# grayhong/self-diagnosing-gan

Hardware: AMD Instinct MI355X
Metric: images/sec (G+D step) (higher is better)
Workload: dtype f32

## Files before the change

### self-diagnosing-gan_amd/csrc/conv_wgrad.hip

```cpp
#include "conv_common.h"
#include "switches.h"
#include <stdlib.h>
#include <type_traits>


namespace diagan {
bool wgrad_wino_supported(int Hi, int Wi, int Ci, int Ho, int Wo, int Co, int R, int S, int sy, int dr, int off, int up,
                          int Kp);
int wgrad_wino_splits(int B, int Ho, int Wo, int Ci, int Co);
int launch_wgrad_wino(WgradArgs a, int splits, int segments, hipStream_t st);
int launch_wgrad_wino_batched(const WgradArgs* jobs, const int* splits, const int* segments, int n, hipStream_t st);
int wgrad_wino_batch_max();
bool wgrad_x3_takes(const WgradArgs& a, bool x3_on);
int launch_wgrad_x3(const WgradArgs& a, int splits, hipStream_t st);
void wgrad_x3_set(int on);


template <int BNn, int BNk, int PRO, bool P2>
__device__ __forceinline__ void conv_wgrad_body(const WgradArgs& a, const int bid, const int nblk) {
  constexpr int BK = 32;
  constexpr int TM = BNn / 64, TN = BNk / 64;
  constexpr int AC = BNn / 4, BC = BNk / 4;
  constexpr int AJ = BK * AC / 256, BJ = BK * BC / 256;
  constexpr int APR = 256 / AC, BPR = 256 / BC;
// ... 356 lines not shown
        for (int u = 0; u < U; ++u)
          t[u][r] = __builtin_bit_cast(f32x4, __builtin_amdgcn_raw_buffer_load_b128(src, voff[u] + (unsigned)r * sbytes, 0, 0));
#pragma unroll
      for (int u = 0; u < U; ++u) {
#pragma unroll
        for (int w = 1; w < R; w <<= 1)
#pragma unroll
          for (int r = 0; r + w < R; r += 2 * w) t[u][r] += t[u][r + w];
        acc[u] += t[u][0];
      }
    }
    if (sn) {
      double dot = 0.0;
      const __amdgpu_buffer_rsrc_t wsrc = __builtin_amdgcn_make_buffer_rsrc(const_cast<float*>(L.W), 0, L.n_w * 4, 0x00020000);
      const __amdgpu_buffer_rsrc_t dst = __builtin_amdgcn_make_buffer_rsrc(sl, 0, L.n_elem * 4, 0x00020000);
      f32x4 wv[U];
#pragma unroll
      for (int u = 0; u < U; ++u) wv[u] = __builtin_bit_cast(f32x4, __builtin_amdgcn_raw_buffer_load_b128(wsrc, voff[u], 0, 0));
#pragma unroll
      for (int u = 0; u < U; ++u) {
        const f32x4 g = acc[u];
        if (L.splits > 1)
          __builtin_amdgcn_raw_buffer_store_b128(__builtin_bit_cast(u32x4_t, g), dst, voff[u], 0, 0);
        dot += (double)g[0] * wv[u][0] + (double)g[1] * wv[u][1] + (double)g[2] * wv[u][2] + (double)g[3] * wv[u][3];
        acc[u] = z4;
      }
      dot = wave_sum(dot);
      __syncthreads();
      if ((threadIdx.x & 63) == 0) red[threadIdx.x >> 6] = dot;
      __syncthreads();
      if (threadIdx.x == 0) L.partials[c][lb] = (red[0] + red[1]) + (red[2] + red[3]);
    }
  }
  if (!sn) {
    const __amdgpu_buffer_rsrc_t gsrc = __builtin_amdgcn_make_buffer_rsrc(L.grad, 0, L.n_elem * 4, 0x00020000);
    f32x4 og[U];
#pragma unroll
    for (int u = 0; u < U; ++u) og[u] = __builtin_bit_cast(f32x4, __builtin_amdgcn_raw_buffer_load_b128(gsrc, voff[u], 0, 0));
#pragma unroll
    for (int u = 0; u < U; ++u)
      __builtin_amdgcn_raw_buffer_store_b128(__builtin_bit_cast(u32x4_t, og[u] + acc[u]), gsrc, voff[u], 0, 0);
  }
}

template <typename F>
__device__ __forceinline__ void fin_dispatch(int U, F&& f) {
  switch (U) {
    case 8: f(std::integral_constant<int, 8>{}); break;
    case 4: f(std::integral_constant<int, 4>{}); break;
    case 2: f(std::integral_constant<int, 2>{}); break;
    default: f(std::integral_constant<int, 1>{}); break;
  }
}

__global__ __launch_bounds__(256) __attribute__((amdgpu_waves_per_eu(4, 4))) void wgrad_finish_a_kernel(const WgFinish* __restrict__ tab, int n_layers) {
  const WgFinish L = load_uniform(tab + find_layer(tab, n_layers, blockIdx.x));
  const int lb = blockIdx.x - L.first_block;
  const int U = fin_u(L.splits);
  if ((long)lb * 1024 * U >= L.n_elem) return;
  __shared__ double red[4];
  fin_dispatch(U, [&](auto u) { fin_a<decltype(u)::value>(L, lb, red); });
}

__global__ __launch_bounds__(256) void wgrad_finish_dot_kernel(const WgFinish* __restrict__ tab) {
  const WgFinish L = tab[blockIdx.x];
  if (L.W == nullptr) return;
  __shared__ double red[256];
  const int fe = 1024 * fin_u(L.splits), nparts = (L.n_elem + fe - 1) / fe;
  for (int c = 0; c < L.nctx; ++c) {
    double d = 0.0;
    for (int k = threadIdx.x; k < nparts; k += 256) d += L.partials[c][k];
    red[threadIdx.x] = d;
    __syncthreads();
    for (int w = 128; w > 0; w >>= 1) {
      if ((int)threadIdx.x < w) red[threadIdx.x] += red[threadIdx.x + w];
      __syncthreads();
    }
    if (threadIdx.x == 0) L.partials[c][nparts] = red[0];
    __syncthreads();
  }
}

template <int U>
__device__ __forceinline__ void fin_b(const WgFinish& L, int lb) {
  constexpr int ELEMS = 1024 * U;
  constexpr int UC = U > 1 ? 2 : 1;
  const int nparts = (L.n_elem + ELEMS - 1) / ELEMS;
  float inv[2] = {0.f, 0.f}, coef[2] = {0.f, 0.f};
#pragma unroll
  for (int c = 0; c < 2; ++c) {
    if (c >= L.nctx) break;
    inv[c] = L.state[c][1];
    coef[c] = (float)(L.partials[c][nparts] * (double)inv[c]);
  }
  const int Co = L.n_w / L.Kp;
  const __amdgpu_buffer_rsrc_t gsrc = __builtin_amdgcn_make_buffer_rsrc(L.grad, 0, L.n_elem * 4, 0x00020000);
  __amdgpu_buffer_rsrc_t qsrc[2], vsrc[2], usrc[2];
#pragma unroll
  for (int c = 0; c < 2; ++c) {
    const bool on = c < L.nctx;
    qsrc[c] = __builtin_amdgcn_make_buffer_rsrc(L.slab[c], 0, on ? L.n_elem * 4 : 0, 0x00020000);
    vsrc[c] = __builtin_amdgcn_make_buffer_rsrc(const_cast<float*>(L.v[c]), 0, on ? L.Kp * 4 : 0, 0x00020000);
    usrc[c] = __builtin_amdgcn_make_buffer_rsrc(const_cast<float*>(L.u[c]), 0, on ? Co * 4 : 0, 0x00020000);
  }
#pragma unroll
  for (int u0 = 0; u0 < U; u0 += UC) {
    unsigned po[UC];
    bool okw[UC];
    f32x4 og[UC], gq[UC][2], vv[UC][2];
    float uu[UC][2];
#pragma unroll
    for (int i = 0; i < UC; ++i) {
      const long pos = (long)lb * ELEMS + ((u0 + i) * 256 + threadIdx.x) * 4;
      po[i] = pos < L.n_elem ? (unsigned)pos * 4u : 0x80000000u;
      okw[i] = pos < L.n_w;
      const unsigned n = okw[i] ? (unsigned)pos / (unsigned)L.Kp : 0u;
      const unsigned ko = okw[i] ? ((unsigned)pos - n * (unsigned)L.Kp) * 4u : 0x80000000u;
      const unsigned no = okw[i] ? n * 4u : 0x80000000u;
      og[i] = __builtin_bit_cast(f32x4, __builtin_amdgcn_raw_buffer_load_b128(gsrc, po[i], 0, 0));
#pragma unroll
      for (int c = 0; c < 2; ++c) {
        gq[i][c] = __builtin_bit_cast(f32x4, __builtin_amdgcn_raw_buffer_load_b128(qsrc[c], po[i], 0, 0));
        vv[i][c] = __builtin_bit_cast(f32x4, __builtin_amdgcn_raw_buffer_load_b128(vsrc[c], ko, 0, 0));
        uu[i][c] = __builtin_bit_cast(float, __builtin_amdgcn_raw_buffer_load_b32(usrc[c], no, 0, 0));
      }
    }
#pragma unroll
    for (int i = 0; i < UC; ++i) {
      f32x4 o = og[i];
#pragma unroll
      for (int c = 0; c < 2; ++c) {
        const f32x4 w = (gq[i][c] - (uu[i][c] * coef[c]) * vv[i][c]) * inv[c];
        o += okw[i] ? w : gq[i][c];
      }
      __builtin_amdgcn_raw_buffer_store_b128(__builtin_bit_cast(u32x4_t, o),
                                             gsrc, po[i], 0, 0);
    }
    __builtin_amdgcn_sched_barrier(0);
  }
}

__global__ __launch_bounds__(256) void wgrad_finish_b_kernel(const WgFinish* __restrict__ tab, int n_layers) {
  const WgFinish L = load_uniform(tab + find_layer(tab, n_layers, blockIdx.x));
  const int lb = blockIdx.x - L.first_block;
  const int U = fin_u(L.splits);
  if (L.W == nullptr || (long)lb * 1024 * U >= L.n_elem) return;
  fin_dispatch(U, [&](auto u) { fin_b<decltype(u)::value>(L, lb); });
}

extern "C" __attribute__((visibility("default"))) int diagan_wgrad_finish_block_elems(int splits) { return 1024 * fin_u(splits); }

}

using namespace diagan;
extern "C" int diagan_conv_gemm_get_wino(void);
extern "C" int diagan_conv_gemm_get_x3b(void);
extern "C" int diagan_conv_wgrad_splits(int M, int Co, int Kp);
extern "C" int diagan_conv_wgrad_uses_wino(int Hi, int Wi, int Ci, int Ho, int Wo, int Co, int R, int S, int sy, int dr,
                                           int off, int up, int Kp);

DIAGAN_API int diagan_wgrad_finish_batched(const void* table_dev, int n_layers, int64_t total_blocks, int any_sn,
                                           void* stream) {
  DG_REQUIRE(table_dev && n_layers > 0 && total_blocks > 0 && total_blocks < (1L << 31), "wgrad_finish_batched: bad args");
  static_assert(sizeof(WgFinish) == 128, "descriptor layout");
  const WgFinish* tab = (const WgFinish*)table_dev;
  hipStream_t st = (hipStream_t)stream;
  hipLaunchKernelGGL(wgrad_finish_a_kernel, dim3((unsigned)total_blocks), dim3(256), 0, st, tab, n_layers);
  if (any_sn) {
    hipLaunchKernelGGL(wgrad_finish_dot_kernel, dim3(n_layers), dim3(256), 0, st, tab);
    hipLaunchKernelGGL(wgrad_finish_b_kernel, dim3((unsigned)total_blocks), dim3(256), 0, st, tab, n_layers);
  }
  return check_launch("wgrad_finish_batched");
}

static void wgrad_tile(int Co, int Kp, int* bn, int* bk) {
  *bn = Co <= 64 ? 64 : 128;
  *bk = Kp <= 64 ? 64 : 128;
  if (*bn == 128 && *bk == 64) *bn = 64;
}

static void wgrad_gemm_fields(WgradArgs& a, int* bn, int* bk, bool* p2) {
  const ConvGeom& g = a.g;
  wgrad_tile(g.Co, g.Kp, bn, bk);
  a.tiles = cdiv(g.Co, *bn) * cdiv(g.Kp, *bk);
  a.same = (g.Hi == g.Ho && g.Wi == g.Wo && g.sy == 1 && g.up == 1) ? 1 : 0;
  *p2 = (g.Ho & (g.Ho - 1)) == 0 && (g.Wo & (g.Wo - 1)) == 0;
  a.lgW = a.lgHW = 0;
  while ((1 << a.lgW) < g.Wo) ++a.lgW;
  while ((1 << a.lgHW) < g.Ho * g.Wo) ++a.lgHW;
}

static int wgrad_fill_args(WgradArgs& a, const float* dy, const float* x, float* slab, int splits, int segments,
                           int64_t slab_stride, int64_t bias_off, const float* pro_scale, const float* pro_shift, int pro_mode, int B,
                           int Hi, int Wi, int Ci, int Ho, int Wo, int Co, int R, int S, int sy, int dr, int off, int up, int Kp) {
  DG_REQUIRE(dy && x && slab, "conv_wgrad: null tensor");
  DG_REQUIRE(B > 0 && Hi > 0 && Wi > 0 && Ho > 0 && Wo > 0 && R > 0 && S > 0, "conv_wgrad: bad dims");
  DG_REQUIRE(Ci > 0 && (Ci & 3) == 0 && Co > 0 && (Co & 3) == 0, "conv_wgrad: Ci=%d, Co=%d must be multiples of 4", Ci, Co);
  DG_REQUIRE(up == 1 || up == 2, "conv_wgrad: up=%d unsupported", up);
  DG_REQUIRE(dr == 1 || dr == -1, "conv_wgrad: dr must be +-1");
  DG_REQUIRE(Kp % 32 == 0 && Kp >= R * S * Ci, "conv_wgrad: bad Kp=%d", Kp);
  DG_REQUIRE(splits >= 1, "conv_wgrad: splits=%d", splits);
  DG_REQUIRE(pro_mode >= 0 && pro_mode <= PRO_BOX_RELU, "conv_wgrad: bad pro_mode %d", pro_mode);
  DG_REQUIRE(!(pro_mode == PRO_BOX || pro_mode == PRO_BOX_RELU) || (up == 1 && dr == 1 && Hi >= 2 && Wi >= 2),
             "conv_wgrad: the box-sum loader (pro_mode 5 / 6) gathers forward geometries without up-sampling");
  DG_REQUIRE(!(pro_mode == PRO_AFFINE_RELU || pro_mode == PRO_AFFINE) || (pro_scale && pro_shift),
             "conv_wgrad: affine prologue needs scale/shift");
  DG_REQUIRE(slab_stride >= (int64_t)Co * Kp && (bias_off < 0 || bias_off + Co <= slab_stride),
             "conv_wgrad: slab_stride=%ld too small for Co*Kp=%ld (+bias)", (long)slab_stride, (long)Co * Kp);
  DG_REQUIRE((long)Co * Kp * 4 < (1L << 31), "conv_wgrad: weight tensor must be smaller than 2 GiB");
  DG_REQUIRE((long)B * Ho * Wo * Co * 4 < (1L << 31) && (long)B * Hi * Wi * Ci * 4 < (1L << 31),
             "conv_wgrad: tensors must be smaller than 2 GiB (32-bit buffer offsets)");
  a.dy = dy; a.x = x; a.slab = slab; a.pro_scale = pro_scale; a.pro_shift = pro_shift; a.pro_mode = pro_mode;
  a.M = B * Ho * Wo;
  a.g = ConvGeom{B, Hi, Wi, Ci, Ho, Wo, Co, R, S, sy, dr, off, up, R * S * Ci, Kp};
  a.dWo = make_fastdiv((unsigned)Wo);
  a.dHo = make_fastdiv((unsigned)Ho);
  a.adv_b = 32 / (Ho * Wo);
  a.adv_y = (32 % (Ho * Wo)) / Wo;
  a.adv_x = (32 % (Ho * Wo)) % Wo;
  const int total_steps = cdiv(a.M, 32);
  DG_REQUIRE(segments >= 1 && splits % segments == 0, "conv_wgrad: splits=%d not a multiple of segments=%d", splits, segments);
  DG_REQUIRE(segments == 1 || (a.M % (32 * segments)) == 0, "conv_wgrad: %d pixels do not split into %d segments of whole K-steps", a.M, segments);
  a.seg_steps = cdiv(total_steps, segments);
  a.splits_per_seg = splits / segments;
  a.steps_per_split = cdiv(a.seg_steps, a.splits_per_seg);
  a.slab_stride = slab_stride;
  a.bias_off = bias_off;
  return DIAGAN_OK;
}

DIAGAN_API int diagan_conv_wgrad(const float* dy, const float* x, float* slab, int splits, int segments,
                                 int64_t slab_stride, int64_t bias_off, const float* pro_scale, const float* pro_shift, int pro_mode, int B,
                                 int Hi, int Wi, int Ci, int Ho, int Wo, int Co, int R, int S, int sy,
                                 int dr, int off, int up, int Kp, void* stream) {
  WgradArgs a;
  const int rc = wgrad_fill_args(a, dy, x, slab, splits, segments, slab_stride, bias_off, pro_scale, pro_shift, pro_mode, B, Hi, Wi, Ci,
                                 Ho, Wo, Co, R, S, sy, dr, off, up, Kp);
  if (rc != DIAGAN_OK) return rc;
  hipStream_t st = (hipStream_t)stream;
  if (diagan_conv_wgrad_uses_wino(Hi, Wi, Ci, Ho, Wo, Co, R, S, sy, dr, off, up, Kp))
    return launch_wgrad_wino(a, splits, segments, st);
  int bn, bk;
  bool p2;
  wgrad_gemm_fields(a, &bn, &bk, &p2);
  if (bn == 128 && bk == 128 && wgrad_x3_takes(a, diagan_conv_gemm_get_x3b() != 0)) return launch_wgrad_x3(a, splits, st);
  const dim3 grid(a.tiles * splits);
#define DG_WG(BN_, PRO_) do { if (p2) hipLaunchKernelGGL((conv_wgrad_kernel<BN_, 128, PRO_, true>), grid, dim3(256), 0, st, a); \
                              else hipLaunchKernelGGL((conv_wgrad_kernel<BN_, 128, PRO_, false>), grid, dim3(256), 0, st, a); } while (0)
#define DG_WG_ALL(BN_) switch (pro_mode) { \
      case PRO_NONE: DG_WG(BN_, PRO_NONE); break; \
      case PRO_RELU: DG_WG(BN_, PRO_RELU); break; \
// ... 156 lines not shown
```

### self-diagnosing-gan_amd/diagan/models/base.py

```python
import os

import torch

from diagan.models.layers import FlatNet
from diagan.ops import eltwise as E


PREFETCH_FAKES = os.environ.get("DIAGAN_PREFETCH_FAKES", "1") != "0"
STACK_G_STEP = os.environ.get("DIAGAN_STACK_G_STEP", "1") != "0"


def _world_size():
    from diagan.trainer import distributed as dist
    return dist.get_world_size()


class BaseModel(FlatNet):

    def restore_checkpoint(self, ckpt_file, optimizer=None):
        if not ckpt_file:
            raise ValueError("No checkpoint file to be restored.")
        ckpt_dict = torch.load(ckpt_file, map_location='cpu', weights_only=False)
        self.load_state_dict(ckpt_dict['model_state_dict'])
        self.param_version += 1
# ... 73 lines not shown
            return
        noise = [torch.randn((batch_size, self.nz), device=device) for _ in range(count)]
        for lo in range(0, count, per_chunk):
            part = noise[lo: lo + per_chunk]
            imgs, _ = self.forward_nhwc(torch.cat(part), True, save=False, groups=len(part))
            self._fake_pool.extend(imgs.split(batch_size))
        self._fake_pool_version = self.param_version

    def _take_prefetched(self, num_images):
        pool = getattr(self, '_fake_pool', None)
        if not pool:
            return None
        if pool[0].shape[0] != num_images or self._fake_pool_version != self.param_version or not self.training:
            self._fake_pool = []
            return None
        return pool.pop(0)

    def compute_gan_loss(self, output):
        k = None
        if getattr(self, 'use_topk', False):
            k = int(self.topk_rate * output.shape[0])
        errG, _ = E.loss_gen(output.detach().contiguous(), self.loss_type, k=k, need_grad=False)
        return errG[0]

    def adversarial_grads(self, real_batch, netD, optG, device=None, noise=None):
        self.zero_grad()
        self.wgrad_batch.hold = _world_size() > 1
        batch_size = real_batch[0].shape[0]
        fake, gctx = self.generate_images_nhwc(batch_size, device=device, noise=noise, save=True)
        output, dctx = netD.forward_nhwc(fake, netD.training, save=True, need_dgrad=True, need_in_dgrad=True)
        k = None
        if getattr(self, 'use_topk', False):
            k = int(self.topk_rate * batch_size)
        errG, dlogit = E.loss_gen(output, self.loss_type, k=k)
        g_img = netD.backward_nhwc(dctx, dlogit, need_wgrad=False, need_gx=True)
        self.backward_nhwc(gctx, g_img)
        self.sync_grads(optG)
        return errG

    def train_step(self, real_batch, netD, optG, log_data, device=None, global_step=None, scaler=None, noise=None,
                   **kwargs):
        if scaler is not None:
            raise NotImplementedError("amp/GradScaler is not part of the fp32 MI355X path")
        errG = self.adversarial_grads(real_batch, netD, optG, device=device, noise=noise)
        optG.step()
        log_data.add_metric('errG', errG[0], group='loss')
        return log_data


class BaseDiscriminator(BaseModel):
    supports_defer_step = True

    def __init__(self, ndf, loss_type, **kwargs):
        super().__init__()
        self.ndf, self.loss_type = ndf, loss_type
        self.use_gold = False

    def to_nhwc(self, x):
        return E.nchw_to_nhwc(x.to(dtype=torch.float32), self.in_channels_padded)

    def forward(self, x):
        logit, _ = self.forward_nhwc(self.to_nhwc(x), self.training, save=False, need_dgrad=False)
        return logit

    def compute_gan_loss(self, output_real, output_fake):
        out3, _, _ = E.loss_dis(output_real.detach().contiguous(), output_fake.detach().contiguous(),
                                self.loss_type, gold=self.use_gold, need_grad=False)
        return out3[0]

    def compute_probs(self, output_real, output_fake):
        out3, _, _ = E.loss_dis(output_real.detach().contiguous(), output_fake.detach().contiguous(),
                                self.loss_type, gold=False, need_grad=False)
        return out3[1].item(), out3[2].item()

    def train_step(self, real_batch, netG, optD, log_data, device=None, global_step=None, scaler=None, noise=None,
                   **kwargs):
        if scaler is not None:
            raise NotImplementedError("amp/GradScaler is not part of the fp32 MI355X path")
        self.zero_grad()
        self.wgrad_batch.hold = _world_size() > 1
        real_images = real_batch[0]
        batch_size = real_images.shape[0]
        if getattr(self, 'pair_forward', False) and self.training:
            B, _, H, W = real_images.shape
            x_all = torch.empty((2 * B, H, W, self.in_channels_padded), dtype=torch.float32, device=real_images.device)
            E.nchw_to_nhwc(real_images.to(dtype=torch.float32), self.in_channels_padded, out=x_all[:B])
            netG.generate_images_nhwc(batch_size, device=device, noise=noise, save=False, out=x_all[B:])
            out_all, ctx = self.forward_nhwc(x_all, True, save=True, need_dgrad=True, need_in_dgrad=False, slot='pair')
            dl = torch.empty(2 * B, dtype=torch.float32, device=x_all.device)
            out3, _, _ = E.loss_dis(out_all[:B], out_all[B:], self.loss_type, gold=self.use_gold, d_real=dl[:B],
                                    d_fake=dl[B:])
            self.backward_nhwc(ctx, dl, need_wgrad=True, need_gx=False)
        else:
            out_real, ctx_r = self.forward_nhwc(self.to_nhwc(real_images), self.training, save=True, need_dgrad=True,
                                                need_in_dgrad=False)
            fake, _ = netG.generate_images_nhwc(batch_size, device=device, noise=noise, save=False)
            out_fake, ctx_f = self.forward_nhwc(fake, self.training, save=True, need_dgrad=True, need_in_dgrad=False,
                                                slot=1)
            out3, d_real, d_fake = E.loss_dis(out_real, out_fake, self.loss_type, gold=self.use_gold)
            self.backward_nhwc(ctx_r, d_real, need_wgrad=True, need_gx=False)
            self.backward_nhwc(ctx_f, d_fake, need_wgrad=True, need_gx=False)
        defer = bool(kwargs.get('defer_step', False))
        self.sync_grads(optD, async_op=defer)
        if not defer:
            optD.step()
        log_data.add_metric('errD', out3[0], group='loss')
        log_data.add_metric('D(x)', out3[1], group='prob')
        log_data.add_metric('D(G(z))', out3[2], group='prob')
        return log_data
```

### self-diagnosing-gan_amd/diagan/models/sngan.py

```python
import math

import torch.nn as nn

from diagan.models.base import BaseDiscriminator, BaseGenerator
from diagan.models.layers import BatchNorm, ConvLayer, HeadLinear, LatentLinear, SNBatch
from diagan.ops import conv as C
from diagan.ops import eltwise as E

RELU = (C.PRO_RELU, None, None)


def _bn_pro(bn):
    return (C.PRO_AFFINE_RELU, bn.scale, bn.shift, bn.group_imgs)


class GBlock(nn.Module):
    def __init__(self, in_channels, out_channels, hidden_channels=None, upsample=False):
        super().__init__()
        hidden_channels = hidden_channels if hidden_channels is not None else out_channels
        self.learnable_sc = in_channels != out_channels or upsample
        self.upsample = upsample
        self.c1 = ConvLayer('conv', in_channels, hidden_channels, 3, 1, 1)
        self.c2 = ConvLayer('conv', hidden_channels, out_channels, 3, 1, 1)
        self.b1 = BatchNorm(in_channels)
# ... 68 lines not shown
class DBlock(nn.Module):

    def __init__(self, in_channels, out_channels, hidden_channels=None, downsample=False):
        super().__init__()
        hidden_channels = hidden_channels if hidden_channels is not None else in_channels
        self.downsample = downsample
        self.learnable_sc = (in_channels != out_channels) or downsample
        self.c1 = ConvLayer('conv', in_channels, hidden_channels, 3, 1, 1, sn=True)
        self.c2 = ConvLayer('conv', hidden_channels, out_channels, 3, 1, 1, sn=True)
        self.c1.xavier_(math.sqrt(2.0))
        self.c2.xavier_(math.sqrt(2.0))
        if self.learnable_sc:
            self.c_sc = ConvLayer('conv', in_channels, out_channels, 1, 1, 0, sn=True)
            self.c_sc.xavier_(1.0)

    def forward(self, x, training, save=True, need_dgrad=True, slot=None):
        k1 = self.c1.prepare(training, need_dgrad, slot)
        k2 = self.c2.prepare(training, need_dgrad, slot)
        h1 = self.c1.fwd(k1, x, pro=RELU)
        xp = None
        lo_ok = (x.shape[0] * (x.shape[1] // 2) * (x.shape[2] // 2)) % 64 == 0
        if self.learnable_sc and self.downsample and lo_ok:
            ksc = self.c_sc.prepare(training, need_dgrad, slot)
            xp = E.avgpool2(x, relu_in=True)
            sc = self.c_sc.fwd(ksc, xp)
            out = self.c2.fwd_pool(k2, h1, pro=RELU, residual=sc)
        elif self.learnable_sc:
            ksc = self.c_sc.prepare(training, need_dgrad, slot)
            sc = self.c_sc.fwd(ksc, x, pro=RELU)
            h2 = self.c2.fwd(k2, h1, pro=RELU, residual=sc)
            out = E.avgpool2(h2) if self.downsample else h2
        else:
            ksc = None
            h2 = self.c2.fwd(k2, h1, pro=RELU, residual=x, res_relu=True)
            out = E.avgpool2(h2) if self.downsample else h2
        ctx = dict(x=x, xp=xp, h1=h1, k1=k1, k2=k2, ksc=ksc, slot=0 if slot is None else slot) if save else {}
        return out, ctx

    def backward(self, ctx, gout, need_wgrad=True, need_gx=True):
        x, xp, h1, slot = ctx['x'], ctx['xp'], ctx['h1'], ctx['slot']
        hw = x.shape[1:3]
        unpool = self.downsample and self.c2.dgrad_unpool_fused(gout.shape[0], hw)
        pooled_w = self.downsample and need_wgrad and self.c2.wgrad_pooled_ok(gout, h1)
        lo_path = xp is not None
        need_full = self.downsample and ((need_wgrad and not pooled_w) or not unpool or not lo_path)
        g_full = E.avgpool2_bwd(gout) if need_full else gout
        if pooled_w:
            self.c2.wgrad_pooled(ctx['k2'], gout, h1, relu_in=True, slot=slot)
        elif need_wgrad:
            self.c2.wgrad(ctx['k2'], g_full, h1, pro=RELU, slot=slot)
        if unpool:
            g_h1 = self.c2.dgrad_unpool(ctx['k2'], gout, hw, mask_src=h1)
        else:
            g_h1 = self.c2.dgrad(ctx['k2'], g_full, hw, mask_src=h1)
        if need_wgrad:
            self.c1.wgrad(ctx['k1'], g_h1, x, pro=RELU, slot=slot)
            if xp is not None:
                self.c_sc.wgrad(ctx['ksc'], gout, xp, slot=slot)
            elif self.learnable_sc:
                self.c_sc.wgrad(ctx['ksc'], g_full, x, pro=RELU, slot=slot)
        if not need_gx:
            return None
        if xp is not None:
            g_xp = self.c_sc.dgrad(ctx['ksc'], gout, xp.shape[1:3])
            if self.c1.dgrad_res_unpool_fused(x.shape[0], hw):
                return self.c1.dgrad(ctx['k1'], g_h1, hw, residual=g_xp, mask_src=x, res_unpool=True)
            return self.c1.dgrad(ctx['k1'], g_h1, hw, residual=E.avgpool2_bwd(g_xp), mask_src=x)
        if self.learnable_sc:
            tmp = self.c_sc.dgrad(ctx['ksc'], g_full, hw)
            return self.c1.dgrad(ctx['k1'], g_h1, hw, residual=tmp, mask_src=x)
        return self.c1.dgrad(ctx['k1'], g_h1, hw, residual=g_full, mask_src=x)


class DBlockOptimized(nn.Module):
    def __init__(self, in_channels, out_channels):
        super().__init__()
        self.c1 = ConvLayer('conv', in_channels, out_channels, 3, 1, 1, sn=True)
        self.c2 = ConvLayer('conv', out_channels, out_channels, 3, 1, 1, sn=True)
        self.c_sc = ConvLayer('conv', in_channels, out_channels, 1, 1, 0, sn=True)
        self.c1.xavier_(math.sqrt(2.0))
        self.c2.xavier_(math.sqrt(2.0))
        self.c_sc.xavier_(1.0)

    def forward(self, x, training, save=True, need_dgrad=True, need_in_dgrad=False, slot=None):
        k1 = self.c1.prepare(training, need_dgrad and need_in_dgrad, slot)
        k2 = self.c2.prepare(training, need_dgrad, slot)
        ksc = self.c_sc.prepare(training, need_dgrad and need_in_dgrad, slot)
        h1 = self.c1.fwd(k1, x)
        xp = E.avgpool2(x)
        sc = self.c_sc.fwd(ksc, xp)
        out = self.c2.fwd_pool(k2, h1, pro=RELU, residual=sc)
        ctx = dict(x=x, xp=xp, h1=h1, k1=k1, k2=k2, ksc=ksc, slot=0 if slot is None else slot) if save else {}
        return out, ctx

    def backward(self, ctx, gout, need_wgrad=True, need_gx=True):
        x, xp, h1, slot = ctx['x'], ctx['xp'], ctx['h1'], ctx['slot']
        hw = x.shape[1:3]
        unpool = self.c2.dgrad_unpool_fused(gout.shape[0], hw)
        pooled_w = need_wgrad and self.c2.wgrad_pooled_ok(gout, h1)
        g_full = E.avgpool2_bwd(gout) if ((need_wgrad and not pooled_w) or not unpool) else None
        if need_wgrad:
            self.c_sc.wgrad(ctx['ksc'], gout, xp, slot=slot)
            if pooled_w:
                self.c2.wgrad_pooled(ctx['k2'], gout, h1, relu_in=True, slot=slot)
            else:
                self.c2.wgrad(ctx['k2'], g_full, h1, pro=RELU, slot=slot)
        if unpool:
            g_h1 = self.c2.dgrad_unpool(ctx['k2'], gout, hw, mask_src=h1)
        else:
            g_h1 = self.c2.dgrad(ctx['k2'], g_full, hw, mask_src=h1)
        if need_wgrad:
            self.c1.wgrad(ctx['k1'], g_h1, x, slot=slot)
        if not need_gx:
            return None
        g_xp = self.c_sc.dgrad(ctx['ksc'], gout, xp.shape[1:3])
        g_sc_full = E.avgpool2_bwd(g_xp)
        return self.c1.dgrad(ctx['k1'], g_h1, hw, residual=g_sc_full)


class SNGANBaseGenerator(BaseGenerator):
    out_channels = 3
    supports_stacked_forward = True

    def _blocks(self):
        raise NotImplementedError

    def forward_nhwc(self, z, training, save=True, out=None, groups=1, save_group=None):
        z = z.to(dtype=self.l1.weight.dtype)
        self.wino_batch(('f', None)).prepare(self.param_version)
        x0, h = self.l1.fwd(z)
        bctx = []
        blocks = self._blocks()
        bn = None
        for i, blk in enumerate(blocks):
            nxt = blocks[i + 1].b1 if i + 1 < len(blocks) else self._last_bn
            h, c, bn = blk.forward(h, training, save=save, need_dgrad=save, bn1=bn, next_bn=nxt, groups=groups,
                                   save_group=save_group)
            bctx.append(c)
        k = self._last_conv.prepare(training, need_dgrad=save)
        y_pre = self._last_conv.fwd(k, h, pro=_bn_pro(bn))
        y = E.tanh_fwd(y_pre, out=out)
        if save and groups > 1:
            b = z.shape[0] // groups
            sl = slice(save_group * b, (save_group + 1) * b)
            ctx = dict(x0=x0[sl], bctx=bctx, h=h[sl], bn=E.bn_ctx_group(bn, save_group), k=k, y=y[sl])
        else:
            ctx = dict(x0=x0, bctx=bctx, h=h, bn=bn, k=k, y=y) if save else None
        return y, ctx

    def backward_nhwc(self, ctx, g_img):
        g_pre = E.tanh_bwd(ctx['y'], g_img)
        self.wino_batch(('d', None)).prepare(self.param_version)
        h = ctx['h']
        self._last_conv.wgrad(ctx['k'], g_pre, h, pro=_bn_pro(ctx['bn']))
        g_a = self._last_conv.dgrad(ctx['k'], g_pre, h.shape[1:3])
        g = self._last_bn.bwd(g_a, h, ctx['bn'], relu=True)
        for blk, c in zip(reversed(self._blocks()), reversed(ctx['bctx'])):
            g = blk.backward(c, g)
        self.l1.wgrad(ctx['x0'], g)
        self.wgrad_batch.finish(0)


class SNGANGenerator32(SNGANBaseGenerator):
    max_stacked_images = 1536

    def __init__(self, nz=128, ngf=256, bottom_width=4, loss_type='hinge', **kwargs):
        super().__init__(nz=nz, ngf=ngf, bottom_width=bottom_width, loss_type=loss_type, **kwargs)
        self.l1 = LatentLinear(nz, ngf, bottom_width)
        self.block2 = GBlock(ngf, ngf, upsample=True)
        self.block3 = GBlock(ngf, ngf, upsample=True)
        self.block4 = GBlock(ngf, ngf, upsample=True)
        self.b5 = BatchNorm(ngf)
        self.c5 = ConvLayer('conv', ngf, 3, 3, 1, 1)
        self.l1.xavier_(1.0)
        self.c5.xavier_(1.0)
        self._link_layers()

    def _blocks(self):
        return [self.block2, self.block3, self.block4]

    @property
    def _last_bn(self):
        return self.b5

    @property
    def _last_conv(self):
        return self.c5


class SNGANGenerator64(SNGANBaseGenerator):
    max_stacked_images = 768

    def __init__(self, nz=128, ngf=1024, bottom_width=4, loss_type='hinge', **kwargs):
        super().__init__(nz=nz, ngf=ngf, bottom_width=bottom_width, loss_type=loss_type, **kwargs)
        self.l1 = LatentLinear(nz, ngf, bottom_width)
        self.block2 = GBlock(ngf, ngf >> 1, upsample=True)
        self.block3 = GBlock(ngf >> 1, ngf >> 2, upsample=True)
        self.block4 = GBlock(ngf >> 2, ngf >> 3, upsample=True)
        self.block5 = GBlock(ngf >> 3, ngf >> 4, upsample=True)
        self.b6 = BatchNorm(ngf >> 4)
        self.c6 = ConvLayer('conv', ngf >> 4, 3, 3, 1, 1)
        self.l1.xavier_(1.0)
        self.c6.xavier_(1.0)
        self._link_layers()

    def _blocks(self):
        return [self.block2, self.block3, self.block4, self.block5]

    @property
    def _last_bn(self):
        return self.b6

    @property
    def _last_conv(self):
        return self.c6


class SNGANBaseDiscriminator(BaseDiscriminator):
    in_channels_padded = 4
    pair_forward = True

    def _blocks(self):
        raise NotImplementedError

    def _sn_prepare(self, slot, training, need_dgrad):
        sb = getattr(self, '_sn_batch', None)
        if sb is None or sb.stale():
            layers = [m for m in self.modules() if isinstance(m, ConvLayer) and m.sn] + [self._head]
            sb = SNBatch(self, layers)
            object.__setattr__(self, '_sn_batch', sb)
        if slot == 'pair':
            sb.run_pair(training, need_dgrad)
        else:
            sb.run(slot, training, 1 if need_dgrad else 0)

    def forward_nhwc(self, x, training, save=True, need_dgrad=True, need_in_dgrad=True, slot=0):
        self._sn_prepare(slot, training, need_dgrad)
        self.wino_batch(('f', slot)).prepare(self._wino_version(slot))
        blocks = self._blocks()
        h, c0 = blocks[0].forward(x, training, save=save, need_dgrad=need_dgrad, need_in_dgrad=need_in_dgrad,
                                  slot=slot)
        bctx = [c0]
        for blk in blocks[1:]:
            h, c = blk.forward(h, training, save=save, need_dgrad=need_dgrad, slot=slot)
            bctx.append(c)
        hctx, logit = self._head.fwd(h, training, slot=slot)
        return logit, (dict(bctx=bctx, hctx=hctx, slot=slot) if save else None)

    def _wino_version(self, slot):
        sb = self._sn_batch
        return ('p', self.param_version) if slot == 'pair' else sb.slot_ver.get(slot)

    def backward_nhwc(self, ctx, dlogit, need_wgrad=True, need_gx=False):
        self.wino_batch(('d', ctx['slot'])).prepare(self._wino_version(ctx['slot']))
        g = self._head.bwd(ctx['hctx'], dlogit, need_wgrad=need_wgrad)
        blocks = self._blocks()
        for i in range(len(blocks) - 1, -1, -1):
            g = blocks[i].backward(ctx['bctx'][i], g, need_wgrad=need_wgrad, need_gx=(need_gx or i > 0))
        if need_wgrad:
            self.wgrad_batch.finish(ctx['slot'])
        return g


class SNGANDiscriminator32(SNGANBaseDiscriminator):
    def __init__(self, ndf=128, loss_type='hinge', **kwargs):
        super().__init__(ndf=ndf, loss_type=loss_type, **kwargs)
        self.block1 = DBlockOptimized(3, ndf)
        self.block2 = DBlock(ndf, ndf, downsample=True)
        self.block3 = DBlock(ndf, ndf, downsample=False)
        self.block4 = DBlock(ndf, ndf, downsample=False)
        self.l5 = HeadLinear(ndf, sn=True)
        self.l5.xavier_(1.0)
        self._link_layers()

    def _blocks(self):
        return [self.block1, self.block2, self.block3, self.block4]

    @property
    def _head(self):
        return self.l5


class SNGANDiscriminator64(SNGANBaseDiscriminator):
    def __init__(self, ndf=1024, loss_type='hinge', **kwargs):
        super().__init__(ndf=ndf, loss_type=loss_type, **kwargs)
        self.block1 = DBlockOptimized(3, ndf >> 4)
        self.block2 = DBlock(ndf >> 4, ndf >> 3, downsample=True)
        self.block3 = DBlock(ndf >> 3, ndf >> 2, downsample=True)
        self.block4 = DBlock(ndf >> 2, ndf >> 1, downsample=True)
        self.block5 = DBlock(ndf >> 1, ndf, downsample=True)
        self.l6 = HeadLinear(ndf, sn=True)
        self.l6.xavier_(1.0)
        self._link_layers()

    def _blocks(self):
        return [self.block1, self.block2, self.block3, self.block4, self.block5]

    @property
    def _head(self):
        return self.l6
```

### self-diagnosing-gan_amd/diagan/ops/eltwise.py

```python
import torch

from diagan import _native as nat

LOSS_TYPES = {'gan': 0, 'ns': 1, 'hinge': 2, 'wasserstein': 3}
ptr, st = nat.ptr, nat.current_stream


def _f32(shape, dev):
    return torch.empty(shape, dtype=torch.float32, device=dev)


_ws = {}
_ws_retired = []


def _workspace(dev, nbytes):
    w = _ws.get(dev.index)
    if w is None or w.numel() < nbytes:
        if w is not None:
            _ws_retired.append(w)
        w = torch.empty(max(int(nbytes), 1 << 20), dtype=torch.uint8, device=dev)
        _ws[dev.index] = w
    return w

# ... 60 lines not shown
    ws = _colred_ws(x.device, Mg, C, groups) if training else None
    if training and groups > 1:
        nat.call("diagan_bn_stats_grouped", ptr(x), Mg, C, groups, ptr(gamma), ptr(beta), eps, momentum, ptr(running_mean),
                 ptr(running_var), ptr(ctx.mean), ptr(ctx.invstd), ptr(ctx.scale), ptr(ctx.shift), ptr(ws), st())
        return ctx
    for g in range(groups):
        o = g * C * 4
        nat.call("diagan_bn_stats", ptr(x) + g * Mg * C * 4, Mg, C, ptr(gamma), ptr(beta), eps, momentum,
                 ptr(running_mean), ptr(running_var), 1 if training else 0, ptr(ctx.mean) + o, ptr(ctx.invstd) + o,
                 ptr(ctx.scale) + o, ptr(ctx.shift) + o, ptr(ws), st())
    return ctx


def bn_stats_fused(partials, tiles, M, gamma, beta, running_mean, running_var, eps=1e-5, momentum=0.1, groups=1,
                   group_imgs=0):
    C = gamma.numel()
    if tiles % groups or M % groups:
        raise RuntimeError(f"bn_stats_fused: {tiles} tiles / {M} rows do not split into {groups} groups")
    tg, Mg = tiles // groups, M // groups
    ctx = _bn_ctx(C, Mg, True, groups, group_imgs, gamma.device)
    splits = nat.fn("diagan_bn_stats_fused_splits")(tg, C, groups)
    ws = torch.empty(groups * splits * 2 * C, dtype=torch.float64, device=gamma.device) if splits > 1 else None
    nat.call("diagan_bn_stats_fused", ptr(partials), tg, Mg, C, ptr(gamma), ptr(beta), eps, momentum,
             ptr(running_mean), ptr(running_var), ptr(ctx.mean), ptr(ctx.invstd), ptr(ctx.scale), ptr(ctx.shift), groups,
             ptr(ws), 0 if ws is None else ws.numel(), st())
    return ctx


def bn_bwd(g, x, ctx, relu, dgamma, dbeta, accumulate, residual=None, slope=0.0, drop=None, drop_scale=1.0):
    dx = torch.empty_like(x)
    coef = _f32((2 * ctx.C,), x.device)
    ws = _colred_ws(x.device, ctx.M, ctx.C)
    nat.call("diagan_bn_bwd", ptr(g), ptr(x), ctx.M, ctx.C, ptr(ctx.scale), ptr(ctx.shift), ptr(ctx.mean),
             ptr(ctx.invstd), 1 if ctx.training else 0, 1 if relu else 0, slope, ptr(drop), drop_scale, ptr(dgamma), ptr(dbeta), 1 if accumulate else 0,
             ptr(residual),
             ptr(dx), ptr(coef), ptr(ws), st())
    return dx


def colsum(x, out, accumulate):
    C = x.shape[-1]
    M = x.numel() // C
    ws = _colred_ws(x.device, M, C)
    nat.call("diagan_colsum", ptr(x), M, C, ptr(out), 1 if accumulate else 0, ptr(ws), st())
    return out


def upsample2x(x, pro=None):
    B, H, W, C = x.shape
    mode, scale, shift, group_imgs = (tuple(pro) + (0,))[:4] if pro is not None else (0, None, None, 0)
    out = _f32((B, 2 * H, 2 * W, C), x.device)
    nat.call("diagan_upsample2x", ptr(x), ptr(out), B, H, W, C, mode, ptr(scale), ptr(shift), group_imgs, st())
    return out


def upsample2x_bwd(g, residual=None):
    B, H2, W2, C = g.shape
    out = _f32((B, H2 // 2, W2 // 2, C), g.device)
    nat.call("diagan_upsample2x_bwd", ptr(g), ptr(out), B, H2 // 2, W2 // 2, C, ptr(residual), st())
    return out


def boxsum2(x, relu_in=False):
    B, H, W, C = x.shape
    out = _f32((B, H + 1, W + 1, C), x.device)
    nat.call("diagan_boxsum2", ptr(x), ptr(out), B, H, W, C, 1 if relu_in else 0, st())
    return out


def avgpool2(x, residual=None, relu_in=False):
    B, H, W, C = x.shape
    out = _f32((B, H // 2, W // 2, C), x.device)
    nat.call("diagan_avgpool2", ptr(x), ptr(out), B, H, W, C, ptr(residual), 1 if relu_in else 0, st())
    return out


def avgpool2_bwd(g, residual=None):
    B, Ho, Wo, C = g.shape
    out = _f32((B, 2 * Ho, 2 * Wo, C), g.device)
    nat.call("diagan_avgpool2_bwd", ptr(g), ptr(out), B, 2 * Ho, 2 * Wo, C, ptr(residual), st())
    return out


def head_fwd(x, w, inv_sigma, bias, inv_sigma1=None):
    B, H, W, C = x.shape
    pooled = _f32((B, C), x.device)
    logit = _f32((B, 1), x.device)
    nat.call("diagan_head_fwd", ptr(x), ptr(w), ptr(inv_sigma), ptr(inv_sigma1), B // 2, ptr(bias), ptr(pooled),
             ptr(logit), B, H * W, C, st())
    return pooled, logit


def head_bwd(dlogit, w, inv_sigma, x, pooled, need_gx=True, need_wgrad=True, dbias=None, accumulate_bias=True,
             inv_sigma1=None):
    B, H, W, C = x.shape
    gx = torch.empty_like(x) if need_gx else None
    G = _f32((C,), x.device) if need_wgrad else None
    dot = torch.empty(1, dtype=torch.float64, device=x.device) if need_wgrad else None
    nat.call("diagan_head_bwd", ptr(dlogit), ptr(w), ptr(inv_sigma), ptr(inv_sigma1), B // 2, ptr(x), ptr(pooled),
             ptr(gx), ptr(G), ptr(dot), ptr(dbias), 1 if accumulate_bias else 0, B, H * W, C, st())
    return gx, G, dot


def act_fwd(x, slope, scale=None, shift=None, drop=None, drop_scale=1.0):
    C = x.shape[-1]
    out = torch.empty_like(x)
    nat.call("diagan_act_fwd", ptr(x), ptr(scale), ptr(shift), slope, ptr(drop), drop_scale, ptr(out), x.numel() // C, C, st())
    return out


def act_bwd(g, x, slope, drop=None, drop_scale=1.0):
    out = torch.empty_like(x)
    nat.call("diagan_act_bwd", ptr(g), ptr(x), slope, ptr(drop), drop_scale, ptr(out), x.numel(), st())
    return out


def linear1_fwd(x, w, bias):
    B, C = x.shape
    logit = _f32((B, 1), x.device)
    nat.call("diagan_linear1_fwd", ptr(x), ptr(w), ptr(bias), ptr(logit), B, C, st())
    return logit


def linear1_wgrad(dlogit, x, dw, dbias):
    B, C = x.shape
    nat.call("diagan_linear1_wgrad", ptr(dlogit), ptr(x), ptr(dw), ptr(dbias), B, C, st())


def linear1_bwd_input(dlogit, w, B, C):
    gx = _f32((B, C), w.device)
    nat.call("diagan_linear1_bwd_input", ptr(dlogit), ptr(w), ptr(gx), B, C, st())
    return gx


def add(a, b, out=None):
    out = torch.empty_like(a) if out is None else out
    nat.call("diagan_add", ptr(a), ptr(b), ptr(out), a.numel(), st())
    return out


def loss_dis(out_real, out_fake, loss_type, gold=False, need_grad=True, d_real=None, d_fake=None):
    dev = out_real.device
    nr, nf = out_real.numel(), out_fake.numel()
    if need_grad and d_real is None:
        d_real, d_fake = _f32((nr,), dev), _f32((nf,), dev)
    out3 = _f32((3,), dev)
    nat.call("diagan_loss_dis", ptr(out_real), nr, ptr(out_fake), nf, LOSS_TYPES[loss_type], 1 if gold else 0,
             ptr(d_real), ptr(d_fake), ptr(out3), st())
    return out3, d_real, d_fake


def loss_gen(out_fake, loss_type, k=None, need_grad=True):
    dev = out_fake.device
    n = out_fake.numel()
    k = n if k is None else k
    d_fake = _f32((n,), dev) if need_grad else None
    out1 = _f32((1,), dev)
    nat.call("diagan_loss_gen", ptr(out_fake), n, k, LOSS_TYPES[loss_type], ptr(d_fake), ptr(out1), st())
    return out1, d_fake


def adam_step(p, g, m, v, lr, beta1, beta2, eps, step, grad_scale=1.0):
    bc1 = 1.0 - beta1 ** step
    bc2_sqrt = (1.0 - beta2 ** step) ** 0.5
    nat.call("diagan_adam_step", ptr(p), ptr(g), ptr(m), ptr(v), p.numel(), lr, beta1, beta2, eps, bc1, bc2_sqrt,
             grad_scale, st())
# ... 9 lines not shown
```

Before: 5292.

## Fuse discriminator front layout, pooling and shortcut conv; fold wgrad dot into finish

Adds a d_front kernel that reads real NCHW images and fake NHWC images directly, writes the combined NHWC input, 2x2-average-pools it and computes the 1x1 shortcut conv in one pass. This replaces the separate layout conversion, concat copy, avgpool and shortcut GEMM launches. Separately, the wgrad finish step now computes the spectral-norm dot reduction inside each finish-b block, removing one kernel launch. The cost is that every block redundantly reduces the per-layer partials.

Measured after the change: 5314, median of 6. No clear change (+0.4%).

```diff
diff --git a/include/diagan_d_front.h b/include/diagan_d_front.h
--- /dev/null
+++ b/include/diagan_d_front.h
@@ -0,0 +1,23 @@
+#ifndef DIAGAN_D_FRONT_H
+#define DIAGAN_D_FRONT_H
+
+#include <stdint.h>
+
+#ifdef __cplusplus
+extern "C" {
+#endif
+
+int diagan_d_front_set_enabled(int mode);
+int diagan_d_front_get_enabled(void);
+int diagan_d_front_supported(int n_real, int n_fake, int C, int H, int W, int Cp, int Co, int Kp);
+int diagan_d_front(const float* real, const float* fake, const float* w, const float* bias, float out_scale, const float* scale0,
+                   const float* scale1, int scale_split, float* x_all, float* xp, float* sc, int n_real, int n_fake, int C, int H,
+                   int W, int Co, int Kp, void* stream);
+
+int diagan_wgrad_finish_set_fused(int mode);
+int diagan_wgrad_finish_get_fused(void);
+
+#ifdef __cplusplus
+}
+#endif
+#endif
diff --git a/self-diagnosing-gan_amd/csrc/conv_wgrad.hip b/self-diagnosing-gan_amd/csrc/conv_wgrad.hip
--- a/self-diagnosing-gan_amd/csrc/conv_wgrad.hip
+++ b/self-diagnosing-gan_amd/csrc/conv_wgrad.hip
@@ -462,7 +462,7 @@
 }
 
 template <int U>
-__device__ __forceinline__ void fin_b(const WgFinish& L, int lb) {
+__device__ __forceinline__ void fin_b(const WgFinish& L, int lb, const double* dots = nullptr) {
   constexpr int ELEMS = 1024 * U;
   constexpr int UC = U > 1 ? 2 : 1;
   const int nparts = (L.n_elem + ELEMS - 1) / ELEMS;
@@ -471,7 +471,7 @@
   for (int c = 0; c < 2; ++c) {
     if (c >= L.nctx) break;
     inv[c] = L.state[c][1];
-    coef[c] = (float)(L.partials[c][nparts] * (double)inv[c]);
+    coef[c] = (float)((dots ? dots[c] : L.partials[c][nparts]) * (double)inv[c]);
   }
   const int Co = L.n_w / L.Kp;
   const __amdgpu_buffer_rsrc_t gsrc = __builtin_amdgcn_make_buffer_rsrc(L.grad, 0, L.n_elem * 4, 0x00020000);
@@ -528,6 +528,40 @@
   fin_dispatch(U, [&](auto u) { fin_b<decltype(u)::value>(L, lb); });
 }
 
+__global__ __launch_bounds__(256) void wgrad_finish_b_dot_kernel(const WgFinish* __restrict__ tab, int n_layers) {
+  const WgFinish L = load_uniform(tab + find_layer(tab, n_layers, blockIdx.x));
+  const int lb = blockIdx.x - L.first_block;
+  const int U = fin_u(L.splits);
+  if (L.W == nullptr || (long)lb * 1024 * U >= L.n_elem) return;
+  __shared__ double red[2][256];
+  __shared__ double dots[2];
+  const int fe = 1024 * U, nparts = (L.n_elem + fe - 1) / fe;
+  const int t = threadIdx.x;
+#pragma unroll
+  for (int c = 0; c < 2; ++c) {
+    double d = 0.0;
+    if (c < L.nctx)
+      for (int k = t; k < nparts; k += 256) d += L.partials[c][k];
+    red[c][t] = d;
+  }
+  __syncthreads();
+  if (t < 64) {
+#pragma unroll
+    for (int c = 0; c < 2; ++c) {
+      if (c >= L.nctx) break;
+      double v = (red[c][t] + red[c][t + 128]) + (red[c][t + 64] + red[c][t + 192]);
+#pragma unroll
+      for (int w = 32; w > 0; w >>= 1) v += __shfl_down(v, w, 64);
+      if (t == 0) {
+        dots[c] = v;
+        if (lb == 0) L.partials[c][nparts] = v;
+      }
+    }
+  }
+  __syncthreads();
+  fin_dispatch(U, [&](auto u) { fin_b<decltype(u)::value>(L, lb, dots); });
+}
+
 extern "C" __attribute__((visibility("default"))) int diagan_wgrad_finish_block_elems(int splits) { return 1024 * fin_u(splits); }
 
 }
@@ -538,6 +572,17 @@
 extern "C" int diagan_conv_wgrad_splits(int M, int Co, int Kp);
 extern "C" int diagan_conv_wgrad_uses_wino(int Hi, int Wi, int Ci, int Ho, int Wo, int Co, int R, int S, int sy, int dr,
                                            int off, int up, int Kp);
+
+static int g_finish_fused = -1;
+static Switch kFinishFused{{"DIAGAN_WGRAD_FINISH_FUSED", 1}};
+static bool finish_fused_on() { return kFinishFused.get(-1, g_finish_fused) != 0; }
+
+DIAGAN_API int diagan_wgrad_finish_set_fused(int mode) {
+  DG_REQUIRE(mode >= -1 && mode <= 1, "wgrad_finish_set_fused: -1, 0 or 1");
+  g_finish_fused = mode;
+  return DIAGAN_OK;
+}
+DIAGAN_API int diagan_wgrad_finish_get_fused(void) { return finish_fused_on() ? 1 : 0; }
 
 DIAGAN_API int diagan_wgrad_finish_batched(const void* table_dev, int n_layers, int64_t total_blocks, int any_sn,
                                            void* stream) {
@@ -546,7 +591,9 @@
   const WgFinish* tab = (const WgFinish*)table_dev;
   hipStream_t st = (hipStream_t)stream;
   hipLaunchKernelGGL(wgrad_finish_a_kernel, dim3((unsigned)total_blocks), dim3(256), 0, st, tab, n_layers);
-  if (any_sn) {
+  if (any_sn && finish_fused_on()) {
+    hipLaunchKernelGGL(wgrad_finish_b_dot_kernel, dim3((unsigned)total_blocks), dim3(256), 0, st, tab, n_layers);
+  } else if (any_sn) {
     hipLaunchKernelGGL(wgrad_finish_dot_kernel, dim3(n_layers), dim3(256), 0, st, tab);
     hipLaunchKernelGGL(wgrad_finish_b_kernel, dim3((unsigned)total_blocks), dim3(256), 0, st, tab, n_layers);
   }
diff --git a/self-diagnosing-gan_amd/csrc/d_front.hip b/self-diagnosing-gan_amd/csrc/d_front.hip
--- /dev/null
+++ b/self-diagnosing-gan_amd/csrc/d_front.hip
@@ -0,0 +1,126 @@
+#include "conv_common.h"
+#include "switches.h"
+#include "diagan_d_front.h"
+
+#pragma clang fp contract(off)
+
+namespace diagan {
+
+constexpr int DF_THREADS = 256, DF_PIX = 64;
+
+struct DFrontArgs {
+  const float *real, *fake, *w, *bias, *scale0, *scale1;
+  float *x_all, *xp, *sc;
+  float out_scale;
+  int scale_split, n_real, C, H, W, Co, Kp, lg_c4, n_pool;
+};
+
+__global__ __launch_bounds__(DF_THREADS) void d_front_kernel(const DFrontArgs a) {
+  __shared__ f32x4 xs[DF_THREADS];
+  __shared__ f32x4 xps[DF_PIX];
+  const int tid = threadIdx.x;
+  const int Ho = a.H >> 1, Wo = a.W >> 1;
+  const int p0 = blockIdx.x * DF_PIX;
+
+  {
+    const int dx = tid & 1, pl = (tid >> 1) & (DF_PIX - 1), dy = tid >> 7;
+    const int p = p0 + pl;
+    f32x4 v = {0.f, 0.f, 0.f, 0.f};
+    if (p < a.n_pool) {
+      const int r = p / Wo, ox = p - r * Wo;
+      const int b = r / Ho, oy = r - b * Ho;
+      const int y = 2 * oy + dy, x = 2 * ox + dx;
+      if (b < a.n_real) {
+        const long hw = (long)a.H * a.W;
+        const float* s = a.real + (long)b * a.C * hw + (long)y * a.W + x;
+#pragma unroll
+        for (int c = 0; c < 4; ++c)
+          if (c < a.C) v[c] = s[c * hw];
+      } else {
+        v = *reinterpret_cast<const f32x4*>(a.fake + (((long)(b - a.n_real) * a.H + y) * a.W + x) * 4);
+      }
+      if (a.x_all) *reinterpret_cast<f32x4*>(a.x_all + (((long)b * a.H + y) * a.W + x) * 4) = v;
+    }
+    xs[tid] = v;
+  }
+  __syncthreads();
+  if (tid < DF_PIX) {
+    const f32x4 a0 = xs[2 * tid], a1 = xs[2 * tid + 1], a2 = xs[2 * DF_PIX + 2 * tid], a3 = xs[2 * DF_PIX + 2 * tid + 1];
+    const f32x4 o = ((a0 + a1) + (a2 + a3)) * 0.25f;
+    xps[tid] = o;
+    if (p0 + tid < a.n_pool) reinterpret_cast<f32x4*>(a.xp)[p0 + tid] = o;
+  }
+  __syncthreads();
+
+  const int c4n = 1 << a.lg_c4, c4 = tid & (c4n - 1);
+  f32x4 wr[4];
+#pragma unroll
+  for (int j = 0; j < 4; ++j) wr[j] = *reinterpret_cast<const f32x4*>(a.w + (long)(c4 * 4 + j) * a.Kp);
+  f32x4 bv = {0.f, 0.f, 0.f, 0.f};
+  if (a.bias) bv = reinterpret_cast<const f32x4*>(a.bias)[c4];
+  const float sc0 = a.scale0 ? a.scale0[0] : a.out_scale, sc1 = a.scale1 ? a.scale1[0] : a.out_scale;
+  const int split = a.scale0 ? a.scale_split : 0x7fffffff;
+  for (int idx = tid; idx < (DF_PIX << a.lg_c4); idx += DF_THREADS) {
+    const int pl = idx >> a.lg_c4, p = p0 + pl;
+    if (p >= a.n_pool) break;
+    const f32x4 x = xps[pl];
+    const float s = p < split ? sc0 : sc1;
+    f32x4 o;
+#pragma unroll
+    for (int j = 0; j < 4; ++j) {
+      float acc = 0.f;
+#pragma unroll
+      for (int c = 0; c < 4; ++c) {
+        acc = fmaf(x[c], wr[j][c], acc);
+        acc += 0.f;
+      }
+      o[j] = fmaf(acc, s, bv[j]);
+    }
+    reinterpret_cast<f32x4*>(a.sc)[((long)p << a.lg_c4) + c4] = o;
+  }
+}
+
+static int g_d_front = -1;
+static Switch kDFront{{"DIAGAN_D_FRONT", 1}};
+
+static bool d_front_ok(long n, int C, int H, int W, int Cp, int Co, int Kp) {
+  if (n <= 0 || C < 1 || C > 4 || Cp != 4 || H < 2 || W < 2 || (H & 1) || (W & 1) || Co < 4 || (Co & 3) || Kp < 4 || (Kp & 3)) return false;
+  const int c4 = Co >> 2;
+  if ((c4 & (c4 - 1)) || c4 > 64) return false;
+  const long limit = 1L << 31;
+  return n * H * W * 16 < limit && n * (H / 2) * (W / 2) * Co * 4 < limit;
+}
+
+}
+
+using namespace diagan;
+
+DIAGAN_API int diagan_d_front_set_enabled(int mode) {
+  DG_REQUIRE(mode >= -1 && mode <= 1, "d_front_set_enabled: -1, 0 or 1");
+  g_d_front = mode;
+  return DIAGAN_OK;
+}
+
+DIAGAN_API int diagan_d_front_get_enabled(void) { return kDFront.get(-1, g_d_front) != 0 ? 1 : 0; }
+
+DIAGAN_API int diagan_d_front_supported(int n_real, int n_fake, int C, int H, int W, int Cp, int Co, int Kp) {
+  return n_real >= 0 && n_fake >= 0 && d_front_ok((long)n_real + n_fake, C, H, W, Cp, Co, Kp) ? 1 : 0;
+}
+
+DIAGAN_API int diagan_d_front(const float* real, const float* fake, const float* w, const float* bias, float out_scale,
+                              const float* scale0, const float* scale1, int scale_split, float* x_all, float* xp, float* sc, int n_real,
+                              int n_fake, int C, int H, int W, int Co, int Kp, void* stream) {
+  DG_REQUIRE(n_real >= 0 && n_fake >= 0 && (n_real == 0 || real) && (n_fake == 0 || fake) && w && xp && sc, "d_front: bad args");
+  DG_REQUIRE((scale0 == nullptr) == (scale1 == nullptr), "d_front: one row scale without the other");
+  if (!d_front_ok((long)n_real + n_fake, C, H, W, 4, Co, Kp))
+    return set_err(DIAGAN_EUNSUP, "d_front: %d + %d images of %d x %d x %d to %d channels (Kp %d) is not a shape of this kernel", n_real,
+                   n_fake, C, H, W, Co, Kp);
+  DFrontArgs a;
+  a.real = real, a.fake = fake, a.w = w, a.bias = bias, a.scale0 = scale0, a.scale1 = scale1;
+  a.x_all = x_all, a.xp = xp, a.sc = sc;
+  a.out_scale = out_scale, a.scale_split = scale_split, a.n_real = n_real, a.C = C, a.H = H, a.W = W, a.Co = Co, a.Kp = Kp;
+  a.lg_c4 = __builtin_ctz((unsigned)(Co >> 2));
+  a.n_pool = (n_real + n_fake) * (H / 2) * (W / 2);
+  hipLaunchKernelGGL(d_front_kernel, dim3(cdiv(a.n_pool, DF_PIX)), dim3(DF_THREADS), 0, (hipStream_t)stream, a);
+  return check_launch("d_front");
+}
diff --git a/self-diagnosing-gan_amd/diagan/_native/d_front_abi.py b/self-diagnosing-gan_amd/diagan/_native/d_front_abi.py
--- /dev/null
+++ b/self-diagnosing-gan_amd/diagan/_native/d_front_abi.py
@@ -0,0 +1,35 @@
+import os
+
+from diagan import _native as nat
+from diagan._native import parse_header
+
+HEADER_PATH = os.path.join(os.path.dirname(nat.HEADER_PATH), "diagan_d_front.h")
+
+_sigs = None
+_bound = {}
+
+
+def signatures():
+    global _sigs
+    if _sigs is None:
+        if not os.path.exists(HEADER_PATH):
+            raise RuntimeError(f"diagan_d_front.h not found at {HEADER_PATH}: the ctypes signatures are read from it "
+                               "(the package runs from a checkout of the repository).")
+        with open(HEADER_PATH) as f:
+            _sigs = parse_header(f.read())
+    return _sigs
+
+
+def fn(name):
+    f = _bound.get(name)
+    if f is None:
+        f = getattr(nat.lib(), name)
+        f.restype, f.argtypes = signatures()[name]
+        _bound[name] = f
+    return f
+
+
+def call(name, *args):
+    rc = fn(name)(*args)
+    if rc != 0:
+        raise RuntimeError(f"{name} failed ({rc}): {nat.last_error()}")
diff --git a/self-diagnosing-gan_amd/diagan/models/base.py b/self-diagnosing-gan_amd/diagan/models/base.py
--- a/self-diagnosing-gan_amd/diagan/models/base.py
+++ b/self-diagnosing-gan_amd/diagan/models/base.py
@@ -179,12 +179,23 @@
         real_images = real_batch[0]
         batch_size = real_images.shape[0]
         if getattr(self, 'pair_forward', False) and self.training:
-            B, _, H, W = real_images.shape
-            x_all = torch.empty((2 * B, H, W, self.in_channels_padded), dtype=torch.float32, device=real_images.device)
-            E.nchw_to_nhwc(real_images.to(dtype=torch.float32), self.in_channels_padded, out=x_all[:B])
-            netG.generate_images_nhwc(batch_size, device=device, noise=noise, save=False, out=x_all[B:])
-            out_all, ctx = self.forward_nhwc(x_all, True, save=True, need_dgrad=True, need_in_dgrad=False, slot='pair')
-            dl = torch.empty(2 * B, dtype=torch.float32, device=x_all.device)
+            B, C, H, W = real_images.shape
+            front_ok = getattr(self, 'front_ok', None)
+            fake = None
+            if front_ok is not None and E.d_front_src(real_images) and front_ok(B, B, C, H, W):
+                fake, _ = netG.generate_images_nhwc(batch_size, device=device, noise=noise, save=False)
+            if fake is not None and tuple(fake.shape) == (B, H, W, self.in_channels_padded) and E.d_front_src(fake):
+                out_all, ctx = self.forward_nhwc(None, True, save=True, need_dgrad=True, need_in_dgrad=False, slot='pair',
+                                                 src=(real_images, fake))
+            else:
+                x_all = torch.empty((2 * B, H, W, self.in_channels_padded), dtype=torch.float32, device=real_images.device)
+                E.nchw_to_nhwc(real_images.to(dtype=torch.float32), self.in_channels_padded, out=x_all[:B])
+                if fake is not None:
+                    x_all[B:].copy_(fake)
+                else:
+                    netG.generate_images_nhwc(batch_size, device=device, noise=noise, save=False, out=x_all[B:])
+                out_all, ctx = self.forward_nhwc(x_all, True, save=True, need_dgrad=True, need_in_dgrad=False, slot='pair')
+            dl = torch.empty(2 * B, dtype=torch.float32, device=real_images.device)
             out3, _, _ = E.loss_dis(out_all[:B], out_all[B:], self.loss_type, gold=self.use_gold, d_real=dl[:B],
                                     d_fake=dl[B:])
             self.backward_nhwc(ctx, dl, need_wgrad=True, need_gx=False)
diff --git a/self-diagnosing-gan_amd/diagan/models/sngan.py b/self-diagnosing-gan_amd/diagan/models/sngan.py
--- a/self-diagnosing-gan_amd/diagan/models/sngan.py
+++ b/self-diagnosing-gan_amd/diagan/models/sngan.py
@@ -174,13 +174,23 @@
         self.c2.xavier_(math.sqrt(2.0))
         self.c_sc.xavier_(1.0)
 
-    def forward(self, x, training, save=True, need_dgrad=True, need_in_dgrad=False, slot=None):
+    def front_ok(self, n_real, n_fake, C, H, W):
+        g = self.c_sc.geom
+        return C <= self.c1.Cip and E.d_front_ok(n_real, n_fake, C, H, W, self.c1.Cip, g.Co, g.Kp)
+
+    def forward(self, x, training, save=True, need_dgrad=True, need_in_dgrad=False, slot=None, src=None):
         k1 = self.c1.prepare(training, need_dgrad and need_in_dgrad, slot)
         k2 = self.c2.prepare(training, need_dgrad, slot)
         ksc = self.c_sc.prepare(training, need_dgrad and need_in_dgrad, slot)
+        bias = None if self.c_sc.bias is None else self.c_sc.bias.data
+        if src is not None:
+            x, xp, sc = E.d_front(src[0], src[1], ksc.wf, bias, row_scale=ksc.row_scale)
+        elif E.d_front_src(x) and self.front_ok(0, x.shape[0], self.c1.in_ch, x.shape[1], x.shape[2]) and x.shape[3] == self.c1.Cip:
+            _, xp, sc = E.d_front(None, x, ksc.wf, bias, row_scale=ksc.row_scale, need_x_all=False)
+        else:
+            xp = E.avgpool2(x)
+            sc = self.c_sc.fwd(ksc, xp)
         h1 = self.c1.fwd(k1, x)
-        xp = E.avgpool2(x)
-        sc = self.c_sc.fwd(ksc, xp)
         out = self.c2.fwd_pool(k2, h1, pro=RELU, residual=sc)
         ctx = dict(x=x, xp=xp, h1=h1, k1=k1, k2=k2, ksc=ksc, slot=0 if slot is None else slot) if save else {}
         return out, ctx
@@ -326,12 +336,15 @@
         else:
             sb.run(slot, training, 1 if need_dgrad else 0)
 
-    def forward_nhwc(self, x, training, save=True, need_dgrad=True, need_in_dgrad=True, slot=0):
+    def front_ok(self, n_real, n_fake, C, H, W):
+        return self._blocks()[0].front_ok(n_real, n_fake, C, H, W)
+
+    def forward_nhwc(self, x, training, save=True, need_dgrad=True, need_in_dgrad=True, slot=0, src=None):
         self._sn_prepare(slot, training, need_dgrad)
         self.wino_batch(('f', slot)).prepare(self._wino_version(slot))
         blocks = self._blocks()
         h, c0 = blocks[0].forward(x, training, save=save, need_dgrad=need_dgrad, need_in_dgrad=need_in_dgrad,
-                                  slot=slot)
+                                  slot=slot, src=src)
         bctx = [c0]
         for blk in blocks[1:]:
             h, c = blk.forward(h, training, save=save, need_dgrad=need_dgrad, slot=slot)
diff --git a/self-diagnosing-gan_amd/diagan/ops/eltwise.py b/self-diagnosing-gan_amd/diagan/ops/eltwise.py
--- a/self-diagnosing-gan_amd/diagan/ops/eltwise.py
+++ b/self-diagnosing-gan_amd/diagan/ops/eltwise.py
@@ -166,6 +166,43 @@
     return out
 
 
+def set_d_front(on):
+    from diagan._native import d_front_abi as dnat
+    dnat.call("diagan_d_front_set_enabled", -1 if on is None else (1 if on else 0))
+
+
+def d_front_ok(n_real, n_fake, C, H, W, Cp, Co, Kp):
+    from diagan._native import d_front_abi as dnat
+    return bool(dnat.fn("diagan_d_front_get_enabled")()) and bool(
+        dnat.fn("diagan_d_front_supported")(n_real, n_fake, C, H, W, Cp, Co, Kp))
+
+
+def d_front_src(t):
+    return t.is_cuda and t.dtype == torch.float32 and t.is_contiguous()
+
+
+def d_front(real, fake, w, bias, row_scale=None, need_x_all=True):
+    from diagan._native import d_front_abi as dnat
+    nr, nf = (0 if real is None else real.shape[0]), (0 if fake is None else fake.shape[0])
+    C, H, W = (real.shape[1:]) if real is not None else (3,) + tuple(fake.shape[1:3])
+    n, dev, Co, Kp = nr + nf, w.device, w.shape[0], w.shape[1]
+    if need_x_all or real is not None:
+        x_all = _f32((n, H, W, 4), dev)
+    else:
+        x_all = None
+    xp, sc = _f32((n, H // 2, W // 2, 4), dev), _f32((n, H // 2, W // 2, Co), dev)
+    from diagan.ops import conv as _conv
+    timer = _conv.TIMER
+    t0 = timer.begin("d_front_kernel") if timer is not None else None
+    dnat.call("diagan_d_front", ptr(real), ptr(fake), ptr(w), ptr(bias), 1.0, ptr(row_scale[0]) if row_scale else None,
+              ptr(row_scale[1]) if row_scale else None, (n // 2) * (H // 2) * (W // 2) if row_scale else 0, ptr(x_all), ptr(xp),
+              ptr(sc), nr, nf, C, H, W, Co, Kp, st())
+    if t0 is not None:
+        M = n * (H // 2) * (W // 2)
+        timer.end("d_front_kernel", 2.0 * M * Co * 4, t0, (M, Co, 4, "pro0"))
+    return (fake if x_all is None else x_all), xp, sc
+
+
 def head_fwd(x, w, inv_sigma, bias, inv_sigma1=None):
     B, H, W, C = x.shape
     pooled = _f32((B, C), x.device)
```
